# duckdb-faiss-ext/duckdb-faiss-ext

Measured on AMD Instinct MI355X. Metric: queries/sec, FlatL2 d=128 N=10000000 nq=10000 k=10, higher is better.
Workload: dtype f32 results (bf16 matrix-pipe coarse filter with a proven bound + exact f32 re-scoring of the candidates); 1 GPU; Flat L2 d=128 N=10000000 nq=10000 k=10; queries_per_call=10000, replicas=1, exchange=none

## Files before the change

### duckdb-faiss-ext_amd/csrc/flat_collect.h

```cpp
#pragma once

#include <cstddef>
#include <cstdint>
#include <vector>

#ifdef __HIPCC__
#define MVS_PLAN_HD __host__ __device__
#else
#define MVS_PLAN_HD
#endif

namespace mvs {

constexpr int CL_SCHED_LEVELS = 12;
constexpr int CL_BODY_MIN_ROWS = 7680;
constexpr int CL_BODY_MAX_RANGES = 384;
constexpr int CL_TAPER_ROUNDS = 2;
constexpr int CL_TAPER_FLOOR_ROWS = 512;
constexpr unsigned CL_ITEM_NONE = 0xffffffffu;

struct CollectSched {
	int nlev, nranges;
	int first[CL_SCHED_LEVELS];
	int rows[CL_SCHED_LEVELS];
// ... 4 lines not shown
	CollectSched s = {};
	if (n_rows <= 0 || stage_rows <= 0)
		return s;
	if (nqb < 1)
		nqb = 1;
	const int64_t total = (n_rows + stage_rows - 1) / stage_rows;
	int64_t nbody = n_rows / CL_BODY_MIN_ROWS;
	nbody = nbody < 1 ? 1 : (nbody > CL_BODY_MAX_RANGES ? CL_BODY_MAX_RANGES : nbody);
	const int64_t body = (total + nbody - 1) / nbody;
	const int64_t per_round = (slots + nqb - 1) / nqb;
	int64_t floor_st = (CL_TAPER_FLOOR_ROWS + stage_rows - 1) / stage_rows;
	if (floor_st < (body + 511) / 512)
		floor_st = (body + 511) / 512;
	int64_t rem = total, size = body, done = 0, nr = 0;
	while (rem > 0) {
		const bool last = size <= floor_st || s.nlev == CL_SCHED_LEVELS - 1;
		int64_t count;
		if (last) {
			count = (rem + size - 1) / size;
		} else {
			const int64_t keep = (int64_t)CL_TAPER_ROUNDS * per_round * size;
			count = rem > keep ? (rem - keep + size - 1) / size : 0;
			if (count > rem / size)
				count = rem / size;
		}
		if (count > 0) {
			s.first[s.nlev] = (int)nr;
			s.rows[s.nlev] = (int)(size * stage_rows);
			s.begin[s.nlev] = done * stage_rows;
			++s.nlev;
			nr += count;
			done += count * size;
			rem = last ? 0 : rem - count * size;
		}
		size = (size + 1) / 2 > floor_st ? (size + 1) / 2 : floor_st;
	}
	s.nranges = (int)nr;
	return s;
}
inline std::vector<int64_t> collect_plan_ranges(int64_t n_rows, int64_t stage_rows, int64_t nqb, int64_t slots) {
	const CollectSched s = collect_plan_levels(n_rows, stage_rows, nqb, slots);
	std::vector<int64_t> b;
	for (int l = 0; l < s.nlev; ++l) {
		const int end = l + 1 < s.nlev ? s.first[l + 1] : s.nranges;
		for (int r = s.first[l]; r < end; ++r)
			b.push_back(s.begin[l] + (int64_t)(r - s.first[l]) * s.rows[l]);
	}
	b.push_back(n_rows > 0 ? n_rows : 0);
	return b;
}
MVS_PLAN_HD inline int64_t collect_queue_items(int nranges, int x, int64_t nqb) {
	return nranges > x ? (int64_t)((nranges - x + 7) >> 3) * nqb : 0;
}
constexpr int CL_CURSOR_STRIDE = 32;
constexpr size_t CL_CURSOR_BYTES = 9 * CL_CURSOR_STRIDE * 4;

}

#ifndef MVS_COLLECT_PLAN_ONLY
#include "flat_fused.h"

#include <cstddef>

namespace mvs {

typedef __bf16 bf16x8 __attribute__((ext_vector_type(8)));
typedef float f32x4n __attribute__((ext_vector_type(4)));
typedef float f32x2n __attribute__((ext_vector_type(2)));
typedef int i32x4n __attribute__((ext_vector_type(4)));
typedef int i32x2n __attribute__((ext_vector_type(2)));
typedef __attribute__((address_space(3))) float lds_f32c;
typedef __attribute__((address_space(1))) const float glb_f32c;

constexpr int CL_QBLOCK = 512;
constexpr int CL_BN = 32;
constexpr double CL_MFMA_UNITS = 8.0;
constexpr int CL_SUB = 2;
constexpr int CL_SUB_I8 = 4;
constexpr int cl_sub(bool i8) { return i8 ? CL_SUB_I8 : CL_SUB; }
constexpr int CL_QCAP = 2048;
constexpr int cl_qcap(bool i8) { return i8 ? CL_QCAP / 2 : CL_QCAP; }
constexpr int CL_FLUSH_EVERY = 2;
constexpr int CL_FROZEN = 256;

struct CollectArgs {
	const void *qf;
	const unsigned short *yb;
	const float *yn;
	const float *e2;
	unsigned *gslot;
	unsigned long long *stream;
	unsigned long long *stream_cnt;
	float *stream_s;
	float *seed_stage;
	const unsigned long long *rowmask;
	long long stream_cap;
	int slot_stride, nclass;
	long long n, row_first, split_rows;
	long long split_len;
	int nq, nqb, nsplit, xcd_map;
	float *pbnd;
	int flags;
	float i8_unit;
	unsigned *cursors;
};
struct CollectLaunch {
// ... 78 lines not shown
```

### duckdb-faiss-ext_amd/csrc/flat_collect.hip

```cpp
#include "flat_collect.h"

#include <algorithm>
#include <climits>
#include <cmath>
#include <cstring>
#include <type_traits>

#include <rocprim/device/device_radix_sort.hpp>
#include <rocprim/device/device_segmented_radix_sort.hpp>

namespace mvs {

__global__ __launch_bounds__(256) void collect_colsum_kernel(const float *__restrict__ src, long long nrows, int dp,
                                                            int interleaved, float *__restrict__ sum) {
	const int g8 = dp / 8, rl = threadIdx.x / g8, c8 = threadIdx.x % g8, nrl = 256 / g8;
	float acc[8] = {0.f, 0.f, 0.f, 0.f, 0.f, 0.f, 0.f, 0.f};
	const long long r0 = (long long)blockIdx.x * 1024;
	__shared__ float red[256 * 8];
	const bool idle = rl >= nrl;
	for (long long r = r0 + rl; !idle && r < r0 + 1024 && r < nrows; r += nrl) {
		const float4 s0 = *(const float4 *)(src + (size_t)r * dp + c8 * 8);
		const float4 s1 = *(const float4 *)(src + (size_t)r * dp + c8 * 8 + 4);
		float v[8];
		if (!interleaved) {
// ... 612 lines not shown
		const int home = blockIdx.x & 7;
		unsigned dead = qctl[10];
		unsigned got = CL_ITEM_NONE;
		for (int t = 0; t < 8 && got == CL_ITEM_NONE; ++t) {
			const int x = (home + t) & 7;
			if ((dead >> x) & 1u)
				continue;
			const unsigned cnt = (unsigned)collect_queue_items(sc.nranges, x, a.nqb);
			const unsigned j = cnt ? __hip_atomic_fetch_add(cursors + x * CL_CURSOR_STRIDE, 1u, __ATOMIC_RELAXED, __HIP_MEMORY_SCOPE_AGENT) : 0u;
			if (cnt && j < cnt)
				got = (j << 3) | (unsigned)x;
			else
				dead |= 1u << x;
		}
		qctl[10] = dead;
		return got;
	};
	struct Item {
		long long rb, re;
		int qb, rng;
	};
	auto decode = [&](unsigned w) {
		Item it;
		const unsigned x = w & 7u, j = w >> 3;
		const unsigned rr = j / (unsigned)a.nqb;
		it.qb = __builtin_amdgcn_readfirstlane((int)(j - rr * (unsigned)a.nqb));
		it.rng = __builtin_amdgcn_readfirstlane((int)(rr * 8u + x));
		typedef __attribute__((address_space(4))) const CollectSched csched;
		unsigned long long scp = (unsigned long long)(uintptr_t)((__attribute__((address_space(4))) const char *)__builtin_amdgcn_kernarg_segment_ptr() +
		                                                         offsetof(CollectLaunch, sc));
		asm volatile("" : "+s"(scp));
		csched *p = (csched *)(uintptr_t)scp;
		const int nlev = p->nlev;
		int lev = 0;
#pragma unroll 1
		for (int l = 1; l < nlev && it.rng >= p->first[l]; ++l)
			lev = l;
		const int f = p->first[lev], rw = p->rows[lev];
		const long long bg = p->begin[lev];
		it.rb = a.row_first + bg + (long long)(it.rng - f) * rw;
		it.re = it.rb + rw < a.n ? it.rb + rw : a.n;
		return it;
	};
	if (tid == 0) {
		qctl[7] = 0u;
		qctl[10] = 0u;
		qctl[8] = take();
	}
	__syncthreads();
	unsigned curw = (unsigned)__builtin_amdgcn_readfirstlane((int)qctl[8]);
	int hw = 0;
	long long r_begin = 0, r_end = 0;
	int qb = -1;
	int qw = 0;
	frag_t bq[8][KB];

	unsigned dma_off;
	{
		const int rr = I8 ? 8 * wave + (lane >> 3) : 4 * wave + (lane >> 4);
		dma_off = (unsigned)(rr * PITCH + (((lane & (C - 1)) ^ (rr & (C - 1))) * 16));
	}
	auto dma_issue = [&](long long row, int par, int i) {
		const char *base = (const char *)a.yb + (size_t)row * PITCH + (size_t)i * 4096;
		__builtin_amdgcn_global_load_lds((glb_f32c *)(base + dma_off),
		                                 (lds_f32c *)(smem + (par * STAGE_BYTES + (i * 4 + wave) * 1024) / 4), 16, 0, 0);
	};
	auto dma_norms = [&](long long row, int par) {
		const float *base = a.yn + row;
#pragma unroll
		for (int j = 0; j < STAGE_ROWS / 64; ++j)
			__builtin_amdgcn_global_load_lds((glb_f32c *)(base + 64 * j + lane),
			                                 (lds_f32c *)(smem + (2 * STAGE_BYTES) / 4 + par * STAGE_ROWS + 64 * j), 4, 0, 0);
	};
	const bool use_tab = a.pbnd != nullptr;
	const bool frozen = use_tab && (a.flags & CL_FROZEN) != 0;
	constexpr int tab_shift = I8 ? 1 : 2;
	constexpr int duty_mask = (!COLLECT ? 3 : (NC > 32 ? 255 : 63)) >> (I8 ? 1 : 0);
	bool tab_pending = false;
	const float inv_unit = I8 ? 1.0f / unit : 0.f;
	auto dma_bounds = [&](int qbx) {
		const float *base = a.pbnd + (size_t)qbx * CL_QBLOCK + wave * 128;
		float *dst = cqstage + wave * 128;
		__builtin_amdgcn_global_load_lds((glb_f32c *)(base + lane), (lds_f32c *)dst, 4, 0, 16 );
		__builtin_amdgcn_global_load_lds((glb_f32c *)(base + 64 + lane), (lds_f32c *)(dst + 64), 4, 0, 16);
		tab_pending = true;
	};
	auto tab_cvt = [&]() {
		if (!tab_pending)
			return;
		tab_pending = false;
		const float p0 = cqstage[wave * 128 + lane], p1 = cqstage[wave * 128 + 64 + lane];
		if (I8) {
			((int *)cqtab)[wave * 128 + lane] = cl_i8_thr(p0, inv_unit);
			((int *)cqtab)[wave * 128 + 64 + lane] = cl_i8_thr(p1, inv_unit);
		} else {
			cqtab[wave * 128 + lane] = p0;
			cqtab[wave * 128 + 64 + lane] = p1;
		}
	};

	const unsigned rbase = (unsigned)(c * PITCH) | (unsigned)(((hq ^ c) & (C - 1)) * 16);
	constexpr int WQCAP = QCAP / 4;
	const unsigned qcnt_lds = (unsigned)(uintptr_t)((__attribute__((address_space(3))) unsigned *)qctl);
	const unsigned qbuf_lds = (unsigned)(uintptr_t)((__attribute__((address_space(3))) unsigned long long *)qbuf) + (unsigned)(wave * WQCAP * 8);
	const unsigned qval_lds = (unsigned)(uintptr_t)((__attribute__((address_space(3))) float *)qval) + (unsigned)(wave * WQCAP * 4);
	const unsigned cq_lds = (unsigned)(uintptr_t)((__attribute__((address_space(3))) float *)cqtab) + (unsigned)((wave * 64 + c) * 8);

	int ovf = 0;
	int wfill = 0, wpub = 0;
	auto publish = [&]() __attribute__((always_inline)) {
		const unsigned n = (unsigned)wfill < (unsigned)WQCAP ? (unsigned)wfill : (unsigned)WQCAP;
		for (unsigned e = (unsigned)wpub + lane; e < n && !frozen; e += 64) {
			unsigned long long ent;
			float v;
			asm volatile("ds_read_b64 %0, %2\n\tds_read_b32 %1, %3\n\ts_waitcnt lgkmcnt(0)"
			             : "=&v"(ent), "=&v"(v)
			             : "v"(qbuf_lds + 8u * e), "v"(qval_lds + 4u * e)
			             : "memory");
			const unsigned row = (unsigned)ent;
			typedef __attribute__((address_space(1))) unsigned *GU;
			__hip_atomic_fetch_min((GU)(a.gslot + (size_t)(unsigned)(ent >> 32) * NC) + (row & (unsigned)(NC - 1)), skey(v), __ATOMIC_RELAXED,
			                       __HIP_MEMORY_SCOPE_AGENT);
		}
		wpub = (int)n;
	};
	auto wdrain = [&]() __attribute__((always_inline)) {
		publish();
		const unsigned n = (unsigned)wpub;
		wfill = 0;
		wpub = 0;
		if (!COLLECT || n == 0u)
			return;
		unsigned long long base = 0ull;
		if (lane == 0) {
			const unsigned long long n64 = n;
			typedef __attribute__((address_space(1))) unsigned long long *GUL;
			asm volatile("global_atomic_add_x2 %0, %1, %2, off sc0\n\ts_waitcnt vmcnt(0)"
			             : "=&v"(base)
			             : "v"((GUL)a.stream_cnt), "v"(n64)
			             : "memory");
		}
		const unsigned blo = (unsigned)__builtin_amdgcn_readfirstlane((int)(unsigned)base);
		const unsigned bhi = (unsigned)__builtin_amdgcn_readfirstlane((int)(unsigned)(base >> 32));
		base = ((unsigned long long)bhi << 32) | blo;
		for (unsigned e = lane; e < n; e += 64) {
			unsigned long long ent;
			float v;
			asm volatile("ds_read_b64 %0, %2\n\tds_read_b32 %1, %3\n\ts_waitcnt lgkmcnt(0)"
			             : "=&v"(ent), "=&v"(v)
			             : "v"(qbuf_lds + 8u * e), "v"(qval_lds + 4u * e)
			             : "memory");
			if ((long long)(base + e) < a.stream_cap) {
				typedef __attribute__((address_space(1))) unsigned long long *GUL;
				*((GUL)a.stream + (base + e)) = ent;
				if (a.stream_s)
					a.stream_s[base + e] = v;
			}
		}
		ovf |= (long long)(base + n) >= a.stream_cap ? 1 : 0;
	};
	auto rare = [&](const acc_t (&sv)[2], int rb, int t, bool any_t, bnd_t cqv, long long row0, int nvalid, unsigned rowbits) {
		if (__builtin_expect(__builtin_amdgcn_ballot_w64(any_t) == 0ull, 1))
			return;
		int qo = qw;
		MVS_OPAQUE_VGPR(qo);
		unsigned m0 = 0u, m1 = 0u;
		if (any_t) {
#pragma unroll
			for (int r = 0; r < 4; ++r) {
				const bool in = 16 * rb + 4 * hq + r < nvalid;
				m0 |= (in && sv[0][r] >= cqv[0]) ? 1u << r : 0u;
				m1 |= (in && sv[1][r] >= cqv[1]) ? 1u << r : 0u;
			}
			if (SEL) {
				const unsigned rbits = (rowbits >> (16 * rb + 4 * hq)) & 15u;
				m0 &= rbits;
				m1 &= rbits;
			}
		}
		unsigned m = m0 | (m1 << 4);
		while (__builtin_amdgcn_ballot_w64(m != 0u) != 0ull) {
			const bool has = m != 0u;
			const int j8 = has ? __builtin_ctz(m) : 0;
			m &= m - 1u;
			const int i = j8 >> 2, j = j8 & 3;
			const val_t s0 = i ? sv[1][0] : sv[0][0], s1 = i ? sv[1][1] : sv[0][1], s2 = i ? sv[1][2] : sv[0][2], s3 = i ? sv[1][3] : sv[0][3];
			const val_t lo = (j & 1) ? s1 : s0;
			const val_t hi = (j & 1) ? s3 : s2;
			const float v = I8 ? (float)((j & 2) ? hi : lo) * unit : (float)((j & 2) ? hi : lo);
			const unsigned row = (unsigned)(row0 + 16 * rb + 4 * hq + j);
			const unsigned q = (unsigned)(qo + 32 * t + 16 * i + c);
			if (!(COLLECT && ovf) && __builtin_expect(wfill + (int)__builtin_popcountll(__builtin_amdgcn_ballot_w64(has)) > WQCAP, 0))
				wdrain();
			const bool counting = COLLECT && ovf;
			const unsigned long long act = __builtin_amdgcn_ballot_w64(has && !counting);
			const unsigned pos = (unsigned)wfill + __builtin_amdgcn_mbcnt_hi((unsigned)(act >> 32), __builtin_amdgcn_mbcnt_lo((unsigned)act, 0u));
			wfill = __builtin_amdgcn_readfirstlane(wfill + (int)__builtin_popcountll(act));
			if (has) {
				const unsigned long long ent = ((unsigned long long)q << 32) | row;
				if (__builtin_expect(!counting, 1)) {
					asm volatile("ds_write_b64 %0, %1\n\tds_write_b32 %2, %3" ::"v"(qbuf_lds + 8u * pos), "v"(ent), "v"(qval_lds + 4u * pos), "v"(v) : "memory");
				} else {
					typedef __attribute__((address_space(1))) unsigned *GU;
					__hip_atomic_fetch_min((GU)(a.gslot + (size_t)q * NC) + (row & (unsigned)(NC - 1)), skey(v), __ATOMIC_RELAXED,
					                       __HIP_MEMORY_SCOPE_AGENT);
					const unsigned one = 1u;
					asm volatile("ds_add_u32 %0, %1" ::"v"(qcnt_lds + 28u), "v"(one) : "memory");
				}
			}
		}
	};

	int par = 0;
	bool staged = false;
	while (curw != CL_ITEM_NONE) {
	const Item it = decode(curw);
	const bool newq = it.qb != qb;
	r_begin = it.rb, r_end = it.re, qb = it.qb;
	const int ntiles = (int)((r_end - r_begin + STAGE_ROWS - 1) / STAGE_ROWS);
	qw = qb * CL_QBLOCK + wave * 128;
	if (newq) {
		const frag_t *qsrc = (const frag_t *)a.qf;
#pragma unroll
		for (int cb = 0; cb < 8; ++cb) {
			const size_t qblk16 = (size_t)qb * (CL_QBLOCK / 16) + wave * 8 + cb;
#pragma unroll
			for (int kb = 0; kb < KB; ++kb)
				bq[cb][kb] = qsrc[(qblk16 * KB + kb) * 64 + lane];
		}
	}
	if (!staged) {
#pragma unroll
		for (int i = 0; i < DMA_PER_WAVE; ++i)
			dma_issue(r_begin, par, i);
		dma_norms(r_begin, par);
		if (use_tab && newq)
			dma_bounds(qb);
		__syncthreads();
		tab_cvt();
	}
	const int duty_phase = it.rng * 13 + 5;
	for (int u = 0; u < ntiles; ++u) {
		const bool pull = u + 2 == ntiles || ntiles < 2;
		bool hand = false;
		long long nx_rb = 0;
		int nx_qb = qb;
		if (u == ntiles - 1 && ntiles >= 2) {
			const unsigned nxtw = (unsigned)__builtin_amdgcn_readfirstlane((int)qctl[8 + (hw ^ 1)]);
			hand = nxtw != CL_ITEM_NONE;
			if (hand) {
				const Item nx = decode(nxtw);
				nx_rb = nx.rb, nx_qb = nx.qb;
			}
		}
		const int period = u < 4 ? 1 : (u < 32 ? 8 : (u < 256 ? 32 : 128));
		const bool full = !frozen && (use_tab ? ((u + duty_phase) & duty_mask) == 0 : (u % period) == 0);
		if (use_tab && hand && nx_qb != qb)
			dma_bounds(nx_qb);
		else if (use_tab && !full && u > 0 && (u & ((1 << tab_shift) - 1)) == 0)
			dma_bounds(qb);
		if (full) {
			publish();
			int qo = qw;
			MVS_OPAQUE_VGPR(qo);
			f32x2n v = {0.f, 0.f};
#pragma unroll 1
			for (int i = 0; i < 2; ++i) {
				const int q = qo + 32 * hq + 16 * i + c;
				const int qc = q < a.nq ? q : 0;
				const float e2v = __builtin_nontemporal_load(a.e2 + qc);
				constexpr int SUBN = NC > 32 ? 32 : NC, NSUB = NC / SUBN;
				const int rank = NSUB == 1 ? a.nclass - 1 : (a.nclass + NSUB - 1) / NSUB - 1;
				unsigned kth = 0u;
#pragma unroll 1
				for (int sb = 0; sb < NSUB; ++sb) {
				const unsigned long long *src = (const unsigned long long *)(a.gslot + (size_t)qc * NC + sb * SUBN);
				unsigned long long w[SUBN / 2];
#pragma unroll
				for (int j = 0; j < SUBN / 2; ++j)
					w[j] = __hip_atomic_load(src + j, __ATOMIC_RELAXED, __HIP_MEMORY_SCOPE_AGENT);
#pragma unroll
				for (int j = 0; j < SUBN / 2; ++j)
					asm volatile("" : "+v"(w[j]));
				unsigned key[SUBN];
#pragma unroll
				for (int j = 0; j < SUBN / 2; ++j) {
					key[2 * j] = (unsigned)w[j];
					key[2 * j + 1] = (unsigned)(w[j] >> 32);
				}
#pragma unroll
				for (int kbit = 2; kbit <= SUBN; kbit <<= 1)
#pragma unroll
					for (int jb = kbit >> 1; jb > 0; jb >>= 1)
#pragma unroll
						for (int x0 = 0; x0 < SUBN; ++x0) {
							const int x1 = x0 ^ jb;
							if (x1 > x0) {
								const unsigned lo = key[x0] < key[x1] ? key[x0] : key[x1];
								const unsigned hi = key[x0] < key[x1] ? key[x1] : key[x0];
								const bool asc = (x0 & kbit) == 0;
								key[x0] = asc ? lo : hi;
								key[x1] = asc ? hi : lo;
							}
						}
				unsigned ks = key[0];
#pragma unroll
				for (int j = 1; j < SUBN; ++j)
					ks = (rank == j) ? key[j] : ks;
				kth = ks > kth ? ks : kth;
				}
				const unsigned neutral = skey(-FLT_MAX);
				const float B = skey2f(kth < neutral ? kth : neutral);
				const float bv = q < a.nq ? B - e2v : __uint_as_float(0x7fc00000u);
				v[0] = i == 0 ? bv : v[0];
				v[1] = i == 1 ? bv : v[1];
			}
			if (I8) {
				const i32x2n vi = {cl_i8_thr(v[0], inv_unit), cl_i8_thr(v[1], inv_unit)};
				*(i32x2n *)(cqtab + (wave * 64 + hq * 16 + c) * 2) = vi;
			} else {
				*(f32x2n *)(cqtab + (wave * 64 + hq * 16 + c) * 2) = v;
			}
			if (use_tab) {
				unsigned long long bits;
				__builtin_memcpy(&bits, &v, 8);
				__hip_atomic_store((unsigned long long *)(a.pbnd + (size_t)qb * CL_QBLOCK + (wave * 64 + hq * 16 + c) * 2), bits, __ATOMIC_RELAXED,
				                   __HIP_MEMORY_SCOPE_AGENT);
			}
		}
#pragma unroll 1
		for (int sub = 0; sub < SUB; ++sub) {
		frag_t A[KB][2];
		acc_t Y[2];
		{
			const unsigned nb_lds = (unsigned)(uintptr_t)((lds_f32c *)(nbuf + par * STAGE_ROWS + sub * CL_BN + 4 * hq));
			asm volatile("ds_read_b128 %0, %2\n\tds_read_b128 %1, %2 offset:64" : "=&v"(Y[0]), "=&v"(Y[1]) : "v"(nb_lds) : "memory");
			const unsigned ab =
			    (unsigned)(uintptr_t)((lds_f32c *)(smem + (par * STAGE_BYTES + sub * TILE_BYTES) / 4)) + rbase;
#pragma unroll
			for (int kb = 0; kb < KB; ++kb) {
				asm volatile("ds_read_b128 %0, %1" : "=v"(A[kb][0]) : "v"(ab ^ (unsigned)(kb * 64)) : "memory");
				if (I8)
					asm volatile("ds_read_b128 %0, %1 offset:2048" : "=v"(A[kb][1]) : "v"(ab ^ (unsigned)(kb * 64)) : "memory");
				else
					asm volatile("ds_read_b128 %0, %1 offset:4096" : "=v"(A[kb][1]) : "v"(ab ^ (unsigned)(kb * 64)) : "memory");
			}
		}
		if (sub == 0) {
			const long long nrow = hand ? nx_rb : r_begin + (long long)(u + 1) * STAGE_ROWS;
#pragma unroll
			for (int i = 0; i < DMA_PER_WAVE; ++i)
				dma_issue(nrow, par ^ 1, i);
			dma_norms(nrow, par ^ 1);
		}
		const long long row0 = r_begin + ((long long)u * SUB + sub) * CL_BN;
		const int nvalid = (int)((r_end - row0) < CL_BN ? (r_end - row0) : CL_BN);
		unsigned rowbits = 0xFFFFFFFFu;
		if (SEL) {
			typedef __attribute__((address_space(4))) const unsigned cuint;
			rowbits = *((cuint *)a.rowmask + (row0 >> 5));
		}

		acc_t acc[2][2];
		bnd_t cqv[2];
		const val_t lowest = I8 ? (val_t)INT_MIN : (val_t)-INFINITY;
		val_t mx0 = lowest, mx1 = lowest;
		auto vmax = [](val_t x, val_t y) {
			if constexpr (I8)
				return x > y ? x : y;
			else
				return __builtin_fmaxf(x, y);
		};
		auto fold = [&](acc_t &p, int rb, int i) {
			(void)rb;
			if (i == 0)
				mx0 = vmax(vmax(vmax(vmax(mx0, p[0]), p[1]), p[2]), p[3]);
			else
				mx1 = vmax(vmax(vmax(vmax(mx1, p[0]), p[1]), p[2]), p[3]);
		};
		auto any_of = [&](bnd_t cqp) {
			const bool r = (mx0 >= cqp[0]) || (mx1 >= cqp[1]);
			mx0 = lowest;
			mx1 = lowest;
			return r;
		};
#pragma unroll
		for (int t = 0; t < 4; ++t) {
			asm volatile("ds_read_b64 %0, %1" : "=v"(cqv[t & 1]) : "v"(cq_lds + (unsigned)(t * 128)) : "memory");
#pragma unroll
			for (int rb = 0; rb < 2; ++rb) {
				const int prb = rb ^ 1, pt = rb == 0 ? t - 1 : t;
#pragma unroll
				for (int kb = 0; kb < KB; ++kb) {
					if constexpr (I8) {
						if (t == 0) {
							if (rb == 0 && kb == 0)
								asm volatile("s_waitcnt lgkmcnt(4)" : "+v"(A[0][0]), "+v"(Y[0]), "+v"(Y[1]));
							else if (rb == 0 && kb == 1)
								asm volatile("s_waitcnt lgkmcnt(2)" : "+v"(A[1][0]));
							else if (rb == 1 && kb == 0)
								asm volatile("s_waitcnt lgkmcnt(0)" : "+v"(A[0][1]), "+v"(A[1][1]), "+v"(cqv[0]));
						}
					} else if (t == 0) {
						if (rb == 0 && kb == 0)
							asm volatile("s_waitcnt lgkmcnt(8)" : "+v"(A[0][0]), "+v"(Y[0]), "+v"(Y[1]));
						else if (rb == 0 && kb == 1)
							asm volatile("s_waitcnt lgkmcnt(6)" : "+v"(A[1][0]));
						else if (rb == 0 && kb == 2)
							asm volatile("s_waitcnt lgkmcnt(4)" : "+v"(A[2][0]));
						else if (rb == 0 && kb == 3)
							asm volatile("s_waitcnt lgkmcnt(2)" : "+v"(A[3][0]));
						else if (rb == 1 && kb == 0)
							asm volatile("s_waitcnt lgkmcnt(0)" : "+v"(A[0][1]), "+v"(A[1][1]), "+v"(A[2][1]), "+v"(A[3][1]), "+v"(cqv[0]));
					}
#pragma unroll
					for (int i = 0; i < 2; ++i) {
						if constexpr (I8)
							acc[rb][i] = __builtin_amdgcn_mfma_i32_16x16x64_i8(A[kb][rb], bq[2 * t + i][kb], kb == 0 ? Y[rb] : acc[rb][i], 0, 0, 0);
						else if (kb == 0)
							acc[rb][i] = __builtin_amdgcn_mfma_f32_16x16x32_bf16(A[kb][rb], bq[2 * t + i][kb], Y[rb], 0, 0, 0);
						else
							acc[rb][i] = __builtin_amdgcn_mfma_f32_16x16x32_bf16(A[kb][rb], bq[2 * t + i][kb], acc[rb][i], 0, 0, 0);
					}
					if (pt >= 0 && kb < 2)
						fold(acc[prb][kb], prb, kb);
					__builtin_amdgcn_sched_barrier(0);
				}
				if (pt >= 0) {
					if (rb == 0)
						asm volatile("s_waitcnt lgkmcnt(0)" : "+v"(cqv[0]), "+v"(cqv[1]));
					rare(acc[prb], prb, pt, any_of(cqv[pt & 1]), cqv[pt & 1], row0, nvalid, rowbits);
				}
			}
		}
		{
			fold(acc[1][0], 1, 0);
			fold(acc[1][1], 1, 1);
			rare(acc[1], 1, 3, any_of(cqv[1]), cqv[1], row0, nvalid, rowbits);
		}
		}
		if (pull && tid == 0)
			qctl[8 + (hw ^ 1)] = take();
		__syncthreads();
		tab_cvt();
		par ^= 1;
		constexpr int FLUSH_EVERY = I8 ? CL_FLUSH_EVERY / 2 : CL_FLUSH_EVERY;
		static_assert(FLUSH_EVERY >= 1, "queue cadence");
		if ((u % FLUSH_EVERY) == FLUSH_EVERY - 1 || u == ntiles - 1) {
			if (wfill >= WQCAP / 2)
				wdrain();
			else
				publish();
		}
	}
	curw = (unsigned)__builtin_amdgcn_readfirstlane((int)qctl[8 + (hw ^ 1)]);
	hw ^= 1;
	staged = curw != CL_ITEM_NONE && ntiles >= 2;
	}
	wdrain();
	if (COLLECT) {
		__syncthreads();
		if (tid == 0 && qctl[7] != 0u)
			atomicAdd(a.stream_cnt, (unsigned long long)qctl[7]);
	}
	if (tid == 0) {
		const unsigned done = __hip_atomic_fetch_add(cursors + 8 * CL_CURSOR_STRIDE, 1u, __ATOMIC_RELAXED, __HIP_MEMORY_SCOPE_AGENT);
		if (done == gridDim.x - 1u)
			for (int x = 0; x < 9; ++x)
				__hip_atomic_store(cursors + x * CL_CURSOR_STRIDE, 0u, __ATOMIC_RELAXED, __HIP_MEMORY_SCOPE_AGENT);
	}
}

constexpr size_t cl_lds_bytes(bool i8) {
	return (size_t)2 * cl_sub(i8) * CL_BN * 128 * (i8 ? 1 : 2) + (size_t)2 * cl_sub(i8) * CL_BN * 4 + (size_t)cl_qcap(i8) * 8 + (size_t)CL_QBLOCK * 4 + 64 +
	       (size_t)cl_qcap(i8) * 4 + (size_t)CL_QBLOCK * 4;
}
static_assert(3 * cl_lds_bytes(true) <= 160 * 1024 && 2 * cl_lds_bytes(false) <= 160 * 1024, "LDS per workgroup of the d <= 128 scan");
static size_t collect_lds_bytes(const FlatGeom &g, bool i8) {
	(void)g;
	return cl_lds_bytes(i8);
}

bool collect_supported(const FlatGeom &g) {
	return collect_store_dims(g.d) > 0;
}

__device__ __forceinline__ bool cl_sel_member(const SelectorDev &s, long long id) {
	if (s.kind == MVS_SEL_BITMAP) {
		const unsigned long long u = (unsigned long long)id;
		if ((u >> 3) >= (unsigned long long)s.nbytes)
			return false;
		return (s.bitmap[u >> 3] >> (u & 7)) & 1;
	}
	if (s.kind == MVS_SEL_BATCH) {
		long long lo = 0, hi = s.nids;
		while (lo < hi) {
			const long long mid = (lo + hi) >> 1;
			if (s.sorted_ids[mid] < id)
				lo = mid + 1;
			else
				hi = mid;
		}
		return lo < s.nids && s.sorted_ids[lo] == id;
	}
	return true;
}
__global__ __launch_bounds__(256) void collect_rowmask_kernel(SelectorDev sel, const long long *__restrict__ idmap, long long n,
                                                             long long nwords, unsigned long long *__restrict__ mask) {
	const long long row = (long long)blockIdx.x * blockDim.x + threadIdx.x;
	bool ok = false;
	if (row < n)
		ok = cl_sel_member(sel, idmap ? idmap[row] : row);
	const unsigned long long b = __builtin_amdgcn_ballot_w64(ok);
	if ((threadIdx.x & 63) == 0 && (row >> 6) < nwords)
		mask[row >> 6] = b;
}
size_t collect_rowmask_bytes(int64_t n) {
	return (size_t)((n + 63) / 64 + 64) * 8;
}
void launch_collect_rowmask(SelectorDev sel, const int64_t *d_idmap, int64_t n, unsigned long long *d_mask, hipStream_t st) {
	const long long nwords = (long long)(collect_rowmask_bytes(n) / 8);
	const long long rows = nwords * 64;
	hipLaunchKernelGGL(collect_rowmask_kernel, dim3((unsigned)((rows + 255) / 256)), dim3(256), 0, st, sel,
	                   (const long long *)d_idmap, (long long)n, nwords, d_mask);
	MVS_HIP(hipGetLastError());
}


int flat_mfma_slot_stride(int64_t k);
__global__ void init_gslot_kernel(unsigned *g, long long total, int stride, int k, int is_l2);

template <int NC>
__global__ void collect_bound_table_kernel(const unsigned *__restrict__ gslot, const float *__restrict__ e2, int nclass, int nq,
                                           long long total, float *__restrict__ pbnd) {
	const long long j = (long long)blockIdx.x * blockDim.x + threadIdx.x;
	if (j >= total)
		return;
	const int o = (int)(j & 127), w = (int)((j >> 7) & 3);
	const long long qb = j >> 9;
	const int i = o & 1, c = (o >> 1) & 15, hq = o >> 5;
	const long long q = qb * CL_QBLOCK + w * 128 + 32 * hq + 16 * i + c;
	float bv = __uint_as_float(0x7fc00000u);
	if (q < nq) {
		constexpr int SUBN = NC > 32 ? 32 : NC, NSUB = NC / SUBN;
		const int rank = NSUB == 1 ? nclass - 1 : (nclass + NSUB - 1) / NSUB - 1;
		unsigned kth = 0u;
		for (int sb = 0; sb < NSUB; ++sb) {
			unsigned key[SUBN];
#pragma unroll
			for (int t = 0; t < SUBN; ++t)
				key[t] = gslot[(size_t)q * NC + sb * SUBN + t];
			unsigned ks = 0xffffffffu;
#pragma unroll
			for (int t = 0; t < SUBN; ++t) {
				int less = 0, leq = 0;
#pragma unroll
				for (int s2 = 0; s2 < SUBN; ++s2) {
					less += key[s2] < key[t];
					leq += key[s2] <= key[t];
				}
				if (less <= rank && rank < leq)
					ks = key[t];
			}
			kth = ks > kth ? ks : kth;
		}
		const unsigned neutral = skey(-FLT_MAX);
		const float B = skey2f(kth < neutral ? kth : neutral);
		bv = B - e2[q];
	}
	pbnd[j] = bv;
}
static void launch_collect_bound_table(const CollectArgs &a, int nqb, hipStream_t st) {
	if (!a.pbnd)
		return;
	const long long total = (long long)nqb * CL_QBLOCK;
	const dim3 grid((unsigned)((total + 255) / 256));
	if (a.slot_stride == 128)
		hipLaunchKernelGGL(collect_bound_table_kernel<128>, grid, dim3(256), 0, st, (const unsigned *)a.gslot, a.e2, a.nclass, a.nq, total, a.pbnd);
	else if (a.slot_stride == 32)
		hipLaunchKernelGGL(collect_bound_table_kernel<32>, grid, dim3(256), 0, st, (const unsigned *)a.gslot, a.e2, a.nclass, a.nq, total, a.pbnd);
	else
		hipLaunchKernelGGL(collect_bound_table_kernel<16>, grid, dim3(256), 0, st, (const unsigned *)a.gslot, a.e2, a.nclass, a.nq, total, a.pbnd);
	MVS_HIP(hipGetLastError());
}
size_t collect_bound_table_bytes(int64_t nq) {
	return (size_t)((nq + CL_QBLOCK - 1) / CL_QBLOCK) * CL_QBLOCK * sizeof(float) + 1024 + CL_CURSOR_BYTES;
}
unsigned *collect_cursors(float *d_pbnd, int64_t nq) {
	return (unsigned *)(d_pbnd + (size_t)((nq + CL_QBLOCK - 1) / CL_QBLOCK) * CL_QBLOCK + 256);
}

template <bool COLLECT>
static void launch_collect_range(const FlatGeom &g, int metric, CollectArgs a, int64_t row_first, int64_t row_end, int64_t nq, hipStream_t st,
                                 int *grid_out, int *ranges_out, int64_t *items_out) {
	const int nqb = (int)((nq + CL_QBLOCK - 1) / CL_QBLOCK);
	if (!a.pbnd)
		throw Error("flat_bf16_collect_kernel: no bound table, hence no cursors");
	a.cursors = collect_cursors(a.pbnd, nq);
	if (!tune().cl_tab && !(a.flags & CL_FROZEN))
		a.pbnd = nullptr;
	if (!(a.flags & CL_FROZEN))
		launch_collect_bound_table(a, nqb, st);
	const bool i8 = a.i8_unit > 0.f;
	const int64_t stage_rows = cl_sub(i8) * CL_BN;
	const int64_t slots = i8 ? 768 : 512;
	const CollectSched sc = collect_plan_levels(row_end - row_first, stage_rows, nqb, slots);
	const int64_t items = (int64_t)sc.nranges * nqb;
	if (grid_out)
		*grid_out = 0;
	if (ranges_out)
		*ranges_out = sc.nranges;
	if (items_out)
		*items_out = items;
	if (items <= 0)
		return;
	if (items >= ((int64_t)1 << 28))
		throw Error("flat_bf16_collect_kernel: more items than an item word numbers");
	a.row_first = row_first;
	a.n = row_end;
	a.nqb = nqb;
	a.nsplit = sc.nranges;
	const int grid = (int)std::min<int64_t>(slots, items);
	const size_t lds = collect_lds_bytes(g, i8);
#define MVS_CL_GO(L2, SEL_, NC_)                                                                                        \
	{                                                                                                                  \
		auto kern = i8 ? flat_bf16_collect_kernel<8, L2, COLLECT, SEL_, NC_, true> : flat_bf16_collect_kernel<8, L2, COLLECT, SEL_, NC_>; \
		ensure_dynamic_lds((const void *)kern, lds);                                                                   \
		hipLaunchKernelGGL(kern, dim3(grid), dim3(256), lds, st, CollectLaunch{a, sc});                                \
	}
	if (a.slot_stride == 32 || a.slot_stride == 128) {
#define MVS_CL_NC32(L2, SEL_)                                                                                           \
	{                                                                                                                  \
		if (a.slot_stride == 128)                                                                                      \
			MVS_CL_GO(L2, SEL_, 128)                                                                                   \
		else                                                                                                           \
// ... 219 lines not shown
	return (size_t)64 * (size_t)nq * 16 * sizeof(float);
}

int collect_slot_stride(int kk, int dp1) {
	if (dp1 == 128 && kk > 28)
		return 128;
	if (dp1 > 128 && kk > 32 && collect_wide_max_classes(dp1) >= 128)
		return 128;
	return kk > 16 ? 32 : 16;
}
int collect_max_k(int d) {
	const int dp1 = collect_store_dims(d);
	if (dp1 == 0)
		return 0;
	if (dp1 == 128)
		return 128;
	return collect_wide_max_classes(dp1);
}

template <int NC>
__global__ void collect_final_thr_kernel(const unsigned *__restrict__ gslot, const float *__restrict__ e2, int nclass, long long nq,
                                         float *__restrict__ thr) {
	const long long q = (long long)blockIdx.x * blockDim.x + threadIdx.x;
	if (q >= nq)
		return;
	constexpr int SUBN = NC > 32 ? 32 : NC, NSUB = NC / SUBN;
	const int rank = NSUB == 1 ? nclass - 1 : (nclass + NSUB - 1) / NSUB - 1;
	unsigned kth = 0u;
	for (int sb = 0; sb < NSUB; ++sb) {
		unsigned key[SUBN];
#pragma unroll
		for (int t = 0; t < SUBN; ++t)
			key[t] = gslot[(size_t)q * NC + sb * SUBN + t];
		unsigned ks = 0xffffffffu;
#pragma unroll
		for (int t = 0; t < SUBN; ++t) {
			int less = 0, leq = 0;
#pragma unroll
			for (int s2 = 0; s2 < SUBN; ++s2) {
				less += key[s2] < key[t];
				leq += key[s2] <= key[t];
			}
			if (less <= rank && rank < leq)
				ks = key[t];
		}
		kth = ks > kth ? ks : kth;
	}
	const unsigned neutral = skey(-FLT_MAX);
	const float B = skey2f(kth < neutral ? kth : neutral);
	thr[q] = B - e2[q];
}
__global__ void collect_bound_table_multi_kernel(const unsigned *__restrict__ gslot, long long range_stride, int nranges,
                                                 const float *__restrict__ e2, int nclass, int nq, long long total, float *__restrict__ pbnd,
                                                 int linear) {
	const long long j = (long long)blockIdx.x * blockDim.x + threadIdx.x;
	if (j >= total)
		return;
	const int o = (int)(j & 127), w = (int)((j >> 7) & 3);
	const long long qb = j >> 9;
	const int i = o & 1, c = (o >> 1) & 15, hq = o >> 5;
	const long long q = linear ? j : qb * CL_QBLOCK + w * 128 + 32 * hq + 16 * i + c;
	float bv = __uint_as_float(0x7fc00000u);
	if (q < nq) {
		const int rank = (nclass + 3) / 4 - 1;
		unsigned kth = 0u;
		for (int p = 0; p < nranges; ++p)
			for (int sb = 0; sb < 4; ++sb) {
				unsigned key[32];
#pragma unroll
				for (int t = 0; t < 32; ++t)
					key[t] = gslot[(size_t)p * range_stride + (size_t)q * 128 + sb * 32 + t];
				unsigned ks = 0xffffffffu;
#pragma unroll
				for (int t = 0; t < 32; ++t) {
					int less = 0, leq = 0;
#pragma unroll
					for (int s2 = 0; s2 < 32; ++s2) {
						less += key[s2] < key[t];
						leq += key[s2] <= key[t];
					}
					if (less <= rank && rank < leq)
						ks = key[t];
				}
				kth = ks > kth ? ks : kth;
			}
		const unsigned neutral = skey(-FLT_MAX);
		const float B = skey2f(kth < neutral ? kth : neutral);
		bv = B - e2[q];
	}
	pbnd[j] = bv;
}
__global__ void collect_bound_table_seed_kernel(const float *__restrict__ stage, int nsplit, int rank, const float *__restrict__ e2, int nq,
                                                long long total, float *__restrict__ pbnd) {
	const long long j = (long long)blockIdx.x * blockDim.x + threadIdx.x;
	if (j >= total)
		return;
	const int o = (int)(j & 127), w = (int)((j >> 7) & 3);
	const long long qb = j >> 9;
	const int i = o & 1, c = (o >> 1) & 15, hq = o >> 5;
	const long long q = qb * CL_QBLOCK + w * 128 + 32 * hq + 16 * i + c;
	float bv = __uint_as_float(0x7fc00000u);
	if (q < nq) {
		float T = INFINITY;
		for (int p = 0; p < nsplit; ++p) {
			float v[16];
			const f32x4acc *src = (const f32x4acc *)(stage + ((size_t)p * (size_t)nq + (size_t)q) * 16);
#pragma unroll
			for (int t = 0; t < 4; ++t) {
				const f32x4acc x = src[t];
				v[4 * t] = x[0], v[4 * t + 1] = x[1], v[4 * t + 2] = x[2], v[4 * t + 3] = x[3];
			}
			float b = -INFINITY;
#pragma unroll
			for (int t = 0; t < 16; ++t) {
				const float vt = v[t] == v[t] ? v[t] : -INFINITY;
				int greater = 0, geq = 0;
#pragma unroll
				for (int s2 = 0; s2 < 16; ++s2) {
					const float vs = v[s2] == v[s2] ? v[s2] : -INFINITY;
					greater += vs > vt;
					geq += vs >= vt;
				}
				if (greater <= rank && rank < geq)
					b = vt;
			}
			T = b < T ? b : T;
		}
		const float B = T > -FLT_MAX ? T : -FLT_MAX;
		bv = B - e2[q];
	}
	pbnd[j] = bv;
}
void launch_collect_big_bounds_seed(const FlatGeom &g, int metric, const void *d_qf, const unsigned short *d_rows, const float *d_norms, int64_t n,
                                    int64_t nq, int kf, int nsplits, int64_t split_len, const float *d_e2, float *d_stage,
                                    const unsigned long long *d_rowmask, float *d_pbnd, hipStream_t st, float i8_unit) {
	CollectArgs a;
	memset(&a, 0, sizeof a);
	a.qf = d_qf, a.yb = d_rows, a.yn = d_norms, a.e2 = d_e2;
	a.i8_unit = i8_unit;
	a.nq = (int)nq;
	a.rowmask = d_rowmask;
	a.seed_stage = d_stage;
	const int nqb = (int)((nq + CL_QBLOCK - 1) / CL_QBLOCK);
	a.row_first = 0;
	a.split_rows = (n / nsplits) / 64 * 64;
	a.split_len = std::min<int64_t>(split_len, a.split_rows) / 64 * 64;
	a.n = n / 64 * 64;
	a.nqb = nqb;
	a.nsplit = nsplits;
	const int grid = nqb * nsplits;
	const size_t lds = (size_t)2 * CL_SUB * CL_BN * 256 + 2 * 64 * 4 + 64;
#define MVS_SEED(L2, SL)                                                                                           \
	{                                                                                                              \
		auto kern = a.i8_unit > 0.f ? flat_bf16_seed_kernel<L2, SL, true> : flat_bf16_seed_kernel<L2, SL>;         \
		ensure_dynamic_lds((const void *)kern, lds);                                                               \
		hipLaunchKernelGGL(kern, dim3(grid), dim3(256), lds, st, a);                                               \
	}
	if (metric == METRIC_L2 && a.rowmask)
		MVS_SEED(true, true)
	else if (metric == METRIC_L2)
		MVS_SEED(true, false)
	else if (a.rowmask)
		MVS_SEED(false, true)
	else
		MVS_SEED(false, false)
#undef MVS_SEED
	const int kfp = (kf + nsplits - 1) / nsplits;
	const long long total = (long long)nqb * CL_QBLOCK;
	hipLaunchKernelGGL(collect_bound_table_seed_kernel, dim3((unsigned)((total + 127) / 128)), dim3(128), 0, st, (const float *)d_stage, nsplits,
	                   kfp - 1, d_e2, (int)nq, total, d_pbnd);
	MVS_HIP(hipGetLastError());
}
void launch_collect_big_bounds(const FlatGeom &g, int metric, const void *d_qf, const unsigned short *d_rows, const float *d_norms, int64_t n,
                               int64_t nq, int kf, int nranges, int64_t range_rows, const float *d_e2, unsigned *d_gslot,
                               const unsigned long long *d_rowmask, float *d_pbnd, hipStream_t st, float i8_unit) {
	const long long gtotal = (long long)nranges * nq * 128;
	hipLaunchKernelGGL(init_gslot_kernel, dim3((unsigned)((gtotal + 255) / 256)), dim3(256), 0, st, d_gslot, gtotal, 128, 128, 0 );
	const int kfp = (kf + nranges - 1) / nranges;
	const int nqb = (int)((nq + CL_QBLOCK - 1) / CL_QBLOCK);
	const int dp1 = collect_store_dims(g.d);
	for (int p = 0; p < nranges; ++p) {
		CollectArgs a;
		memset(&a, 0, sizeof a);
		a.qf = d_qf, a.yb = d_rows, a.yn = d_norms, a.e2 = d_e2;
		a.i8_unit = dp1 > 128 ? 0.f : i8_unit;
		a.gslot = d_gslot + (size_t)p * nq * 128;
		a.slot_stride = 128;
		a.nclass = kfp;
		a.nq = (int)nq;
		a.rowmask = d_rowmask;
		const int64_t stride = (n / nranges) / 192 * 192, r0 = (int64_t)p * stride, r1 = std::min<int64_t>(n, r0 + std::min<int64_t>(range_rows, stride));
		if (dp1 > 128) {
			const int nqbw = (int)((nq + collect_wide_qblock(dp1) - 1) / collect_wide_qblock(dp1));
			launch_collect_wide_range(dp1, metric, false, a, r0, r1, std::max<int64_t>(8, std::min<int64_t>(64, 1024 / nqbw)), nq, st, nullptr, nullptr);
		} else {
			a.pbnd = d_pbnd;
			launch_collect_range<false>(g, metric, a, r0, r1, nq, st, nullptr, nullptr, nullptr);
		}
	}
	const long long total = dp1 > 128 ? (long long)nq : (long long)nqb * CL_QBLOCK;
	hipLaunchKernelGGL(collect_bound_table_multi_kernel, dim3((unsigned)((total + 127) / 128)), dim3(128), 0, st, (const unsigned *)d_gslot,
	                   (long long)nq * 128, nranges, d_e2, kfp, (int)nq, total, d_pbnd, dp1 > 128 ? 1 : 0);
	MVS_HIP(hipGetLastError());
}

void launch_collect_final_thr(const unsigned *d_gslot, int d, int kk, const float *d_e2, int64_t nq, float *d_thr, hipStream_t st) {
	if (nq <= 0)
		return;
	const int stride = collect_slot_stride(kk, collect_store_dims(d));
	const dim3 grid((unsigned)((nq + 63) / 64));
	if (stride == 128)
		hipLaunchKernelGGL(collect_final_thr_kernel<128>, grid, dim3(64), 0, st, d_gslot, d_e2, kk, (long long)nq, d_thr);
	else if (stride == 32)
		hipLaunchKernelGGL(collect_final_thr_kernel<32>, grid, dim3(64), 0, st, d_gslot, d_e2, kk, (long long)nq, d_thr);
	else
		hipLaunchKernelGGL(collect_final_thr_kernel<16>, grid, dim3(64), 0, st, d_gslot, d_e2, kk, (long long)nq, d_thr);
	MVS_HIP(hipGetLastError());
}

__global__ void collect_report_kernel(const unsigned long long *__restrict__ hdr, const int *__restrict__ fail_cnt,
                                      const unsigned *__restrict__ maxnorm, int *__restrict__ h_flags,
                                      unsigned long long *__restrict__ h_hdr, int with_cnt) {
	const int t = threadIdx.x;
	if (h_hdr && hdr && t < 32)
		h_hdr[t] = hdr[t];
	if (t == 0) {
		h_flags[8] = *fail_cnt;
		h_flags[9] = (int)*maxnorm;
		if (with_cnt && hdr) {
			const unsigned long long c = hdr[0];
			h_flags[10] = (int)(unsigned)c;
			h_flags[11] = (int)(unsigned)(c >> 32);
		}
	}
}
void launch_collect_report(const void *d_hdr, const int *d_fail_cnt, const unsigned *d_maxnorm, int *h_flags, void *h_hdr, bool with_cnt,
                           hipStream_t st) {
	hipLaunchKernelGGL(collect_report_kernel, dim3(1), dim3(64), 0, st, (const unsigned long long *)d_hdr, d_fail_cnt, d_maxnorm, h_flags,
	                   (unsigned long long *)h_hdr, with_cnt ? 1 : 0);
	MVS_HIP(hipGetLastError());
}

void launch_collect_prepare(const FlatGeom &g, int metric, const void *d_qf, const unsigned short *d_rows, const float *d_norms,
                            int64_t n, int64_t nq, int kk, const float *d_e2, unsigned *d_gslot,
                            unsigned long long *d_stream_cnt, const unsigned long long *d_rowmask, float *d_pbnd, hipStream_t st,
                            bool cnt_zeroed, bool slots_ready, float *d_seed_stage, float i8_unit) {
	const int stride = collect_slot_stride(kk, collect_store_dims(g.d));
	const long long gtotal = (long long)nq * stride;
	if (!slots_ready)
		hipLaunchKernelGGL(init_gslot_kernel, dim3((unsigned)((gtotal + 255) / 256)), dim3(256), 0, st, d_gslot, gtotal, stride, stride,
		                   0 );
	if (!cnt_zeroed)
		MVS_HIP(hipMemsetAsync(d_stream_cnt, 0, 16, st));
	CollectArgs a;
	memset(&a, 0, sizeof a);
// ... 592 lines not shown
```

Measured before the change: 1.047 million queries/s.

## Rebalance partial tail query block columns across waves in collect kernel

Adds a per-wave column layout word for each 512-query block. When the last block is only partly filled and four row sub-tiles are in use, the live 32-query columns are spread across the waves instead of fixed 128-query slices, and a partial-tile path runs MFMAs only for the owned columns. The bound-table kernels now map table slots to queries through the same layout. It also adds a fast path in the candidate-emit routine that skips per-row validity checks on full tiles, and uses immediate LDS offsets for the threshold reads. The aim is to cut wasted MFMA work on padded queries and the load imbalance between waves in the tail block, at the cost of extra indexing logic and a second code variant.

```diff
diff --git a/duckdb-faiss-ext_amd/csrc/flat_collect.h b/duckdb-faiss-ext_amd/csrc/flat_collect.h
--- a/duckdb-faiss-ext_amd/csrc/flat_collect.h
+++ b/duckdb-faiss-ext_amd/csrc/flat_collect.h
@@ -80,6 +80,46 @@
 MVS_PLAN_HD inline int64_t collect_queue_items(int nranges, int x, int64_t nqb) {
 	return nranges > x ? (int64_t)((nranges - x + 7) >> 3) * nqb : 0;
 }
+
+constexpr int CL_QCOLS = 16;
+constexpr unsigned CL_QLAYOUT_FULL_N = 0x924u;
+MVS_PLAN_HD inline int collect_qblock_cols(int nq, int qb) {
+	const int live = nq - qb * 32 * CL_QCOLS;
+	return live >= 32 * CL_QCOLS ? CL_QCOLS : (live <= 0 ? 0 : (live + 31) >> 5);
+}
+MVS_PLAN_HD inline unsigned collect_qblock_wave(int nq, int qb, int sub_tiles, int wave) {
+	const int T = collect_qblock_cols(nq, qb);
+	const int own = T >> 2, r = T & 3, spare = 4 - own;
+	if (T == CL_QCOLS || sub_tiles != 4 || (r == 3 && spare == 1))
+		return (unsigned)(4 * wave) * 0x1111u + 0x3210u + (CL_QLAYOUT_FULL_N << 16);
+	const int pair = wave >> 1, half = wave & 1;
+	unsigned cols = 0xFFFFu;
+	unsigned n = 0x249u * (unsigned)own;
+#define MVS_QB_PUT(slot, col) cols = (cols & ~(15u << (4 * (slot)))) | ((unsigned)(col) << (4 * (slot)))
+	for (int t = 0; t < own; ++t)
+		MVS_QB_PUT(t, own * wave + t);
+	if (r <= spare) {
+		for (int j = 0; j < r; ++j)
+			MVS_QB_PUT(own + j, 4 * own + j);
+		n += (unsigned)r << (3 * wave);
+	} else {
+		MVS_QB_PUT(own, 4 * own + pair);
+		n += 9u << (6 * half);
+		if (r == 3) {
+			MVS_QB_PUT(own + 1, 4 * own + 2);
+			n += 1u << (3 * (2 * half + pair));
+		}
+	}
+#undef MVS_QB_PUT
+	return cols | n << 16;
+}
+MVS_PLAN_HD inline int collect_qblock_slot_col(unsigned word, int slot) {
+	return (int)((word >> (4 * slot)) & 15u);
+}
+MVS_PLAN_HD inline int collect_qblock_ncols(unsigned word, int row_tile) {
+	return (int)((word >> (16 + 3 * row_tile)) & 7u);
+}
+
 constexpr int CL_CURSOR_STRIDE = 32;
 constexpr size_t CL_CURSOR_BYTES = 9 * CL_CURSOR_STRIDE * 4;
 
diff --git a/duckdb-faiss-ext_amd/csrc/flat_collect.hip b/duckdb-faiss-ext_amd/csrc/flat_collect.hip
--- a/duckdb-faiss-ext_amd/csrc/flat_collect.hip
+++ b/duckdb-faiss-ext_amd/csrc/flat_collect.hip
@@ -688,7 +688,7 @@
 	int hw = 0;
 	long long r_begin = 0, r_end = 0;
 	int qb = -1;
-	int qw = 0;
+	unsigned lay = 0u;
 	frag_t bq[8][KB];
 
 	unsigned dma_off;
@@ -779,7 +779,9 @@
 		const unsigned blo = (unsigned)__builtin_amdgcn_readfirstlane((int)(unsigned)base);
 		const unsigned bhi = (unsigned)__builtin_amdgcn_readfirstlane((int)(unsigned)(base >> 32));
 		base = ((unsigned long long)bhi << 32) | blo;
-		for (unsigned e = lane; e < n; e += 64) {
+		for (unsigned e0 = lane; e0 < n; e0 += 64) {
+			unsigned e = e0;
+			MVS_OPAQUE_VGPR(e);
 			unsigned long long ent;
 			float v;
 			asm volatile("ds_read_b64 %0, %2\n\tds_read_b32 %1, %3\n\ts_waitcnt lgkmcnt(0)"
@@ -798,16 +800,26 @@
 	auto rare = [&](const acc_t (&sv)[2], int rb, int t, bool any_t, bnd_t cqv, long long row0, int nvalid, unsigned rowbits) {
 		if (__builtin_expect(__builtin_amdgcn_ballot_w64(any_t) == 0ull, 1))
 			return;
-		int qo = qw;
+		int qo = qb * CL_QBLOCK + 32 * collect_qblock_slot_col(lay, t);
 		MVS_OPAQUE_VGPR(qo);
 		unsigned m0 = 0u, m1 = 0u;
-		if (any_t) {
+		int hq4 = 4 * hq;
+		MVS_OPAQUE_VGPR(hq4);
+		if (any_t && __builtin_expect(nvalid >= CL_BN, 1)) {
 #pragma unroll
 			for (int r = 0; r < 4; ++r) {
-				const bool in = 16 * rb + 4 * hq + r < nvalid;
+				m0 |= sv[0][r] >= cqv[0] ? 1u << r : 0u;
+				m1 |= sv[1][r] >= cqv[1] ? 1u << r : 0u;
+			}
+		} else if (any_t) {
+#pragma unroll
+			for (int r = 0; r < 4; ++r) {
+				const bool in = hq4 < nvalid - 16 * rb - r;
 				m0 |= (in && sv[0][r] >= cqv[0]) ? 1u << r : 0u;
 				m1 |= (in && sv[1][r] >= cqv[1]) ? 1u << r : 0u;
 			}
+		}
+		if (any_t) {
 			if (SEL) {
 				const unsigned rbits = (rowbits >> (16 * rb + 4 * hq)) & 15u;
 				m0 &= rbits;
@@ -825,7 +837,7 @@
 			const val_t hi = (j & 1) ? s3 : s2;
 			const float v = I8 ? (float)((j & 2) ? hi : lo) * unit : (float)((j & 2) ? hi : lo);
 			const unsigned row = (unsigned)(row0 + 16 * rb + 4 * hq + j);
-			const unsigned q = (unsigned)(qo + 32 * t + 16 * i + c);
+			const unsigned q = (unsigned)(qo + 16 * i + c);
 			if (!(COLLECT && ovf) && __builtin_expect(wfill + (int)__builtin_popcountll(__builtin_amdgcn_ballot_w64(has)) > WQCAP, 0))
 				wdrain();
 			const bool counting = COLLECT && ovf;
@@ -854,12 +866,12 @@
 	const bool newq = it.qb != qb;
 	r_begin = it.rb, r_end = it.re, qb = it.qb;
 	const int ntiles = (int)((r_end - r_begin + STAGE_ROWS - 1) / STAGE_ROWS);
-	qw = qb * CL_QBLOCK + wave * 128;
+	lay = (unsigned)__builtin_amdgcn_readfirstlane((int)collect_qblock_wave(a.nq, qb, SUB, wave));
 	if (newq) {
 		const frag_t *qsrc = (const frag_t *)a.qf;
 #pragma unroll
 		for (int cb = 0; cb < 8; ++cb) {
-			const size_t qblk16 = (size_t)qb * (CL_QBLOCK / 16) + wave * 8 + cb;
+			const size_t qblk16 = (size_t)qb * (CL_QBLOCK / 16) + 2 * collect_qblock_slot_col(lay, cb >> 1) + (cb & 1);
 #pragma unroll
 			for (int kb = 0; kb < KB; ++kb)
 				bq[cb][kb] = qsrc[(qblk16 * KB + kb) * 64 + lane];
@@ -897,12 +909,12 @@
 			dma_bounds(qb);
 		if (full) {
 			publish();
-			int qo = qw;
+			int qo = qb * CL_QBLOCK + 32 * collect_qblock_slot_col(lay, hq);
 			MVS_OPAQUE_VGPR(qo);
 			f32x2n v = {0.f, 0.f};
 #pragma unroll 1
 			for (int i = 0; i < 2; ++i) {
-				const int q = qo + 32 * hq + 16 * i + c;
+				const int q = qo + 16 * i + c;
 				const int qc = q < a.nq ? q : 0;
 				const float e2v = __builtin_nontemporal_load(a.e2 + qc);
 				constexpr int SUBN = NC > 32 ? 32 : NC, NSUB = NC / SUBN;
@@ -964,8 +976,8 @@
 				                   __HIP_MEMORY_SCOPE_AGENT);
 			}
 		}
-#pragma unroll 1
-		for (int sub = 0; sub < SUB; ++sub) {
+		auto row_tile = [&](auto partial_tag, const int sub) __attribute__((always_inline)) {
+		constexpr bool PARTIAL = decltype(partial_tag)::value;
 		frag_t A[KB][2];
 		acc_t Y[2];
 		{
@@ -1020,9 +1032,49 @@
 			mx1 = lowest;
 			return r;
 		};
+		if constexpr (PARTIAL) {
+			const int ncol = collect_qblock_ncols(lay, sub);
+			asm volatile("s_waitcnt lgkmcnt(0)" : "+v"(Y[0]), "+v"(Y[1]));
+#pragma unroll
+			for (int kb = 0; kb < KB; ++kb)
+				asm volatile("" : "+v"(A[kb][0]), "+v"(A[kb][1]));
+#pragma unroll 1
+			for (int t = 0; t < ncol; ++t) {
+				asm volatile("ds_read_b64 %0, %1" : "=v"(cqv[0]) : "v"(cq_lds + (unsigned)(t * 128)) : "memory");
+#pragma unroll
+				for (int ts = 0; ts < 4; ++ts)
+					if (t == ts) {
+#pragma unroll
+						for (int rb = 0; rb < 2; ++rb)
+#pragma unroll
+							for (int kb = 0; kb < KB; ++kb)
+#pragma unroll
+								for (int i = 0; i < 2; ++i) {
+									if constexpr (I8)
+										acc[rb][i] = __builtin_amdgcn_mfma_i32_16x16x64_i8(A[kb][rb], bq[2 * ts + i][kb], kb == 0 ? Y[rb] : acc[rb][i], 0, 0, 0);
+									else
+										acc[rb][i] = __builtin_amdgcn_mfma_f32_16x16x32_bf16(A[kb][rb], bq[2 * ts + i][kb], kb == 0 ? Y[rb] : acc[rb][i], 0, 0, 0);
+								}
+					}
+				asm volatile("s_waitcnt lgkmcnt(0)" : "+v"(cqv[0]));
+#pragma unroll
+				for (int rb = 0; rb < 2; ++rb) {
+					fold(acc[rb][0], rb, 0);
+					fold(acc[rb][1], rb, 1);
+					rare(acc[rb], rb, t, any_of(cqv[0]), cqv[0], row0, nvalid, rowbits);
+				}
+			}
+		} else {
 #pragma unroll
 		for (int t = 0; t < 4; ++t) {
-			asm volatile("ds_read_b64 %0, %1" : "=v"(cqv[t & 1]) : "v"(cq_lds + (unsigned)(t * 128)) : "memory");
+			if (t == 0)
+				asm volatile("ds_read_b64 %0, %1" : "=v"(cqv[0]) : "v"(cq_lds) : "memory");
+			else if (t == 1)
+				asm volatile("ds_read_b64 %0, %1 offset:128" : "=v"(cqv[1]) : "v"(cq_lds) : "memory");
+			else if (t == 2)
+				asm volatile("ds_read_b64 %0, %1 offset:256" : "=v"(cqv[0]) : "v"(cq_lds) : "memory");
+			else
+				asm volatile("ds_read_b64 %0, %1 offset:384" : "=v"(cqv[1]) : "v"(cq_lds) : "memory");
 #pragma unroll
 			for (int rb = 0; rb < 2; ++rb) {
 				const int prb = rb ^ 1, pt = rb == 0 ? t - 1 : t;
@@ -1075,6 +1127,16 @@
 			rare(acc[1], 1, 3, any_of(cqv[1]), cqv[1], row0, nvalid, rowbits);
 		}
 		}
+		};
+		if (__builtin_expect((lay >> 16) == CL_QLAYOUT_FULL_N, 1)) {
+#pragma unroll 1
+			for (int sub = 0; sub < SUB; ++sub)
+				row_tile(std::false_type{}, sub);
+		} else {
+#pragma unroll 1
+			for (int sub = 0; sub < SUB; ++sub)
+				row_tile(std::true_type{}, sub);
+		}
 		if (pull && tid == 0)
 			qctl[8 + (hw ^ 1)] = take();
 		__syncthreads();
@@ -1166,16 +1228,19 @@
 int flat_mfma_slot_stride(int64_t k);
 __global__ void init_gslot_kernel(unsigned *g, long long total, int stride, int k, int is_l2);
 
-template <int NC>
-__global__ void collect_bound_table_kernel(const unsigned *__restrict__ gslot, const float *__restrict__ e2, int nclass, int nq,
-                                           long long total, float *__restrict__ pbnd) {
-	const long long j = (long long)blockIdx.x * blockDim.x + threadIdx.x;
-	if (j >= total)
-		return;
+__device__ __forceinline__ long long cl_table_query(long long j, int nq, int sub_tiles) {
 	const int o = (int)(j & 127), w = (int)((j >> 7) & 3);
 	const long long qb = j >> 9;
 	const int i = o & 1, c = (o >> 1) & 15, hq = o >> 5;
-	const long long q = qb * CL_QBLOCK + w * 128 + 32 * hq + 16 * i + c;
+	return qb * CL_QBLOCK + 32 * collect_qblock_slot_col(collect_qblock_wave(nq, (int)qb, sub_tiles, w), hq) + 16 * i + c;
+}
+template <int NC>
+__global__ void collect_bound_table_kernel(const unsigned *__restrict__ gslot, const float *__restrict__ e2, int nclass, int nq,
+                                           long long total, float *__restrict__ pbnd, int sub_tiles) {
+	const long long j = (long long)blockIdx.x * blockDim.x + threadIdx.x;
+	if (j >= total)
+		return;
+	const long long q = cl_table_query(j, nq, sub_tiles);
 	float bv = __uint_as_float(0x7fc00000u);
 	if (q < nq) {
 		constexpr int SUBN = NC > 32 ? 32 : NC, NSUB = NC / SUBN;
@@ -1211,12 +1276,13 @@
 		return;
 	const long long total = (long long)nqb * CL_QBLOCK;
 	const dim3 grid((unsigned)((total + 255) / 256));
+	const int sub = cl_sub(a.i8_unit > 0.f);
 	if (a.slot_stride == 128)
-		hipLaunchKernelGGL(collect_bound_table_kernel<128>, grid, dim3(256), 0, st, (const unsigned *)a.gslot, a.e2, a.nclass, a.nq, total, a.pbnd);
+		hipLaunchKernelGGL(collect_bound_table_kernel<128>, grid, dim3(256), 0, st, (const unsigned *)a.gslot, a.e2, a.nclass, a.nq, total, a.pbnd, sub);
 	else if (a.slot_stride == 32)
-		hipLaunchKernelGGL(collect_bound_table_kernel<32>, grid, dim3(256), 0, st, (const unsigned *)a.gslot, a.e2, a.nclass, a.nq, total, a.pbnd);
+		hipLaunchKernelGGL(collect_bound_table_kernel<32>, grid, dim3(256), 0, st, (const unsigned *)a.gslot, a.e2, a.nclass, a.nq, total, a.pbnd, sub);
 	else
-		hipLaunchKernelGGL(collect_bound_table_kernel<16>, grid, dim3(256), 0, st, (const unsigned *)a.gslot, a.e2, a.nclass, a.nq, total, a.pbnd);
+		hipLaunchKernelGGL(collect_bound_table_kernel<16>, grid, dim3(256), 0, st, (const unsigned *)a.gslot, a.e2, a.nclass, a.nq, total, a.pbnd, sub);
 	MVS_HIP(hipGetLastError());
 }
 size_t collect_bound_table_bytes(int64_t nq) {
@@ -1542,14 +1608,11 @@
 }
 __global__ void collect_bound_table_multi_kernel(const unsigned *__restrict__ gslot, long long range_stride, int nranges,
                                                  const float *__restrict__ e2, int nclass, int nq, long long total, float *__restrict__ pbnd,
-                                                 int linear) {
+                                                 int linear, int sub_tiles) {
 	const long long j = (long long)blockIdx.x * blockDim.x + threadIdx.x;
 	if (j >= total)
 		return;
-	const int o = (int)(j & 127), w = (int)((j >> 7) & 3);
-	const long long qb = j >> 9;
-	const int i = o & 1, c = (o >> 1) & 15, hq = o >> 5;
-	const long long q = linear ? j : qb * CL_QBLOCK + w * 128 + 32 * hq + 16 * i + c;
+	const long long q = linear ? j : cl_table_query(j, nq, sub_tiles);
 	float bv = __uint_as_float(0x7fc00000u);
 	if (q < nq) {
 		const int rank = (nclass + 3) / 4 - 1;
@@ -1581,14 +1644,11 @@
 	pbnd[j] = bv;
 }
 __global__ void collect_bound_table_seed_kernel(const float *__restrict__ stage, int nsplit, int rank, const float *__restrict__ e2, int nq,
-                                                long long total, float *__restrict__ pbnd) {
+                                                long long total, float *__restrict__ pbnd, int sub_tiles) {
 	const long long j = (long long)blockIdx.x * blockDim.x + threadIdx.x;
 	if (j >= total)
 		return;
-	const int o = (int)(j & 127), w = (int)((j >> 7) & 3);
-	const long long qb = j >> 9;
-	const int i = o & 1, c = (o >> 1) & 15, hq = o >> 5;
-	const long long q = qb * CL_QBLOCK + w * 128 + 32 * hq + 16 * i + c;
+	const long long q = cl_table_query(j, nq, sub_tiles);
 	float bv = __uint_as_float(0x7fc00000u);
 	if (q < nq) {
 		float T = INFINITY;
@@ -1658,7 +1718,7 @@
 	const int kfp = (kf + nsplits - 1) / nsplits;
 	const long long total = (long long)nqb * CL_QBLOCK;
 	hipLaunchKernelGGL(collect_bound_table_seed_kernel, dim3((unsigned)((total + 127) / 128)), dim3(128), 0, st, (const float *)d_stage, nsplits,
-	                   kfp - 1, d_e2, (int)nq, total, d_pbnd);
+	                   kfp - 1, d_e2, (int)nq, total, d_pbnd, cl_sub(i8_unit > 0.f));
 	MVS_HIP(hipGetLastError());
 }
 void launch_collect_big_bounds(const FlatGeom &g, int metric, const void *d_qf, const unsigned short *d_rows, const float *d_norms, int64_t n,
@@ -1690,7 +1750,7 @@
 	}
 	const long long total = dp1 > 128 ? (long long)nq : (long long)nqb * CL_QBLOCK;
 	hipLaunchKernelGGL(collect_bound_table_multi_kernel, dim3((unsigned)((total + 127) / 128)), dim3(128), 0, st, (const unsigned *)d_gslot,
-	                   (long long)nq * 128, nranges, d_e2, kfp, (int)nq, total, d_pbnd, dp1 > 128 ? 1 : 0);
+	                   (long long)nq * 128, nranges, d_e2, kfp, (int)nq, total, d_pbnd, dp1 > 128 ? 1 : 0, cl_sub(i8_unit > 0.f));
 	MVS_HIP(hipGetLastError());
 }
 
```

After: 1.058 million queries/s, median of 6. 1.01x the previous value.
